# bytedance/particle-sfm

Hardware: AMD Instinct MI355X
Metric: trajectory-points/s (higher is better)
Workload: dtype f32 sampling + f64 positions; 1 GPU; configs[1]: synthetic 100x(1920x1080) flow pairs, sample_ratio=2, flow_check + chaining + occlusion + id assignment, 1 sequence per GPU; frames=101, height=1080, width=1920, trajectories=2073277, parallelism=sequence-per-gpu x1, world_size=1

## Files before the change

### particle-sfm_amd/csrc/psfm_persist.hip

```cpp
#include <hip/hip_ext.h>
#include <stdlib.h>

#include "psfm_internal.h"
#include "psfm_chain.h"

#define PP_BLOCK 256
#define PP_NW (PP_BLOCK / PSFM_WAVE)
#define PP_PROBE 8
#ifndef PP_PRE_WAVES
#define PP_PRE_WAVES 4
#endif
#ifndef PP_KEEP
#define PP_KEEP 0
#endif
#ifndef PP_FC_AHEAD
#define PP_FC_AHEAD 4
#endif
#ifndef PP_FC_FAST
#define PP_FC_FAST 0
#endif
#define PP_GUESTS 32
#ifndef PP_WHATIF
#define PP_WHATIF 0
#endif
#ifndef PP_WAVES_N
#define PP_WAVES_N 8
#endif
#define PP_WAVES __attribute__((amdgpu_waves_per_eu(PP_WAVES_N, PP_WAVES_N)))

#ifdef PSFM_PERSIST_CHECK
#define PP_CHK(idx, lim, code) (((idx) >= 0 && (idx) < (lim)) ? true : (atomicCAS(&a.ctr->pad[0], 0, (code)), atomicMax(&a.ctr->pad[1], (int)(idx)), false))
#else
#define PP_CHK(idx, lim, code) true
#endif
#ifndef PP_COH_MARKS
#define PP_COH_MARKS true
#endif
#define PP_POOLED (-1)
#define PP_PEND (-2)

struct PsfmPersistArgs {
    const float2* flows; const uint8_t* occ;
    const float2* flows_b; uint8_t* occ_w; float thres, t2; int fc; int fc_xcd_per;
    int xcd_per;
    int64_t occ_pitch; PsfmFastDiv wdiv;
    int H, W; float cw, ch, rcw, rch;
    int ratio, GW, GH, G;
    float2* dlog; int cap;
    int cap_main;
    uint8_t* maps;
    unsigned* survsh;
    PsfmCounters* ctr;
    PsfmShard* shards;
    int* free_stack; int free_cap; int nsh;
    unsigned long long* handoff;
    unsigned long long* fin_keys; int* fin_lanes;
    int seg_cap; int spill_base; int spill_cap;
    int2* seg_info;
    unsigned* bar;
    int n_flows, shift_b, shift_d;
    PsfmFastDiv gwdiv, rdiv;
    int spin_limit;
};

struct PsfmFrameView {
    const float2* flow; const uint8_t* occ;
    int H, W; float cw, ch, rcw, rch;
    int ratio, GW, GH;
    uint8_t* blocked_cur; uint8_t stamp_cur;
    PsfmFastDiv rdiv;
};

__device__ __forceinline__ void psfm_put_record(const PsfmPersistArgs& a, int slot, unsigned long long key, int lane)
{
    int64_t o;
    if (slot < a.seg_cap) {
        o = (int64_t)blockIdx.x * a.seg_cap + slot;
    } else {
        const int q = atomicAdd(&a.ctr->spill_cnt, 1);
        if (q >= a.spill_cap) { atomicOr(&a.ctr->overflow, 2); return; }
        o = (int64_t)a.spill_base + q;
    }
    if (!PP_CHK(lane, a.cap, 6)) return;
    a.fin_keys[o] = key;
    a.fin_lanes[o] = lane;
}

__device__ __forceinline__ int psfm_record_slot(int* s_rec_cnt, bool dead)
{
    const unsigned long long dm = __ballot(dead);
    if (dm == 0ull) return 0;
    int base = 0;
    if (psfm_lane_id() == (int)__builtin_ctzll(dm)) base = atomicAdd(s_rec_cnt, __popcll(dm));
    base = __shfl(base, (int)__builtin_ctzll(dm));
    return base + psfm_rank_in(dm);
}

#ifdef PSFM_TIMELINE
__device__ unsigned long long g_pp_tl[2 * 4096 * 8];
__device__ int g_pp_st[4096 * 8];
__device__ int g_pp_tl_frame = -1;
#define PP_TL(k) do { if ((unsigned)(t - g_pp_tl_frame) < 2u && tid == 0) g_pp_tl[((t - g_pp_tl_frame) * 4096 + blockIdx.x) * 8 + (k)] = __builtin_amdgcn_s_memrealtime(); } while (0)
extern "C" int psfm_debug_persist_timeline(int frame, unsigned long long* out_host, int n_blocks)
{
    if (out_host && n_blocks < 0) return hipMemcpyFromSymbol(out_host, HIP_SYMBOL(g_pp_st), (size_t)(-n_blocks) * 32) != hipSuccess;
    if (out_host) return hipMemcpyFromSymbol(out_host, HIP_SYMBOL(g_pp_tl), (size_t)2 * 4096 * 64) != hipSuccess;
    return hipMemcpyToSymbol(HIP_SYMBOL(g_pp_tl_frame), &frame, sizeof(int)) != hipSuccess;
}
#else
#define PP_TL(k) do {} while (0)
#endif

__device__ __forceinline__ void psfm_bar_arrive(const PsfmPersistArgs& a, int shard, int k, int lane)
{
    int last = 0;
    if (lane == 0) {
        const int nblk = (int)gridDim.x;
        const unsigned members = (unsigned)((nblk - shard + PSFM_NSHARD - 1) / PSFM_NSHARD);
        const unsigned old = __hip_atomic_fetch_add(a.bar + shard * 32, 1u, __ATOMIC_RELAXED, __HIP_MEMORY_SCOPE_AGENT);
        if (old + 1 == members * (unsigned)(k + 1)) {
            const unsigned nsh = (unsigned)(nblk < PSFM_NSHARD ? nblk : PSFM_NSHARD);
            const unsigned o2 = __hip_atomic_fetch_add(a.bar + 64 * 32, 1u, __ATOMIC_RELAXED, __HIP_MEMORY_SCOPE_AGENT);
            if (o2 + 1 == nsh * (unsigned)(k + 1)) last = 1;
        }
    }
    last = __builtin_amdgcn_readfirstlane(last);
    if (last) psfm_coh_st(a.bar + (65 + lane) * 32, (unsigned)(k + 1));
}
__device__ __forceinline__ bool psfm_bar_wait(const PsfmPersistArgs& a, int shard, int k)
{
    const unsigned* flag = a.bar + (65 + shard) * 32;
    int n = 0;
    while (psfm_coh_ld(flag) < (unsigned)(k + 1)) {
        __builtin_amdgcn_s_sleep(1);
        if (++n > a.spin_limit) { atomicOr(&a.ctr->overflow, 8); psfm_coh_st(&a.ctr->abort, 1); return false; }
        if ((n & 127) == 0 && psfm_coh_ld(&a.ctr->abort)) return false;
    }
    return true;
}

__device__ __forceinline__ void psfm_fc_slice(const PsfmPersistArgs& a, int f, int tid)
{
    const int P = a.H * a.W;
    PsfmFcParams q;
    q.H = a.H; q.W = a.W; q.cw = a.cw; q.ch = a.ch; q.rcw = a.rcw; q.rch = a.rch; q.thres = a.thres; q.t2 = a.t2;
    const float2* __restrict__ F = a.flows + (size_t)f * P;
    const float2* __restrict__ B = a.flows_b + (size_t)f * P;
    uint8_t* O = a.occ_w + (size_t)f * a.occ_pitch;
    const int nch = (P + 1023) / 1024;
    const int per = a.fc_xcd_per;
    for (int q0 = blockIdx.x; q0 < (per > 0 ? 8 * per : nch); q0 += gridDim.x) {
        const int ci = per > 0 ? (q0 & 7) * per + (q0 >> 3) : q0;
        if (ci >= nch) continue;
        const int p0 = ci * 1024 + tid;
        float2 fv[4];
#pragma unroll
        for (int k = 0; k < 4; ++k) {
            const int p = p0 + k * 256;
            fv[k] = p < P ? psfm_ld(F, (unsigned)p * 8u) : make_float2(0.f, 0.f);
        }
        int y = (int)psfm_fastdiv((unsigned)p0, a.wdiv), x = p0 - y * a.W;
#pragma unroll
        for (int k = 0; k < 4; ++k) {
            const int p = p0 + k * 256;
            if (p >= P) break;
            uint8_t o;
#if PP_FC_FAST
            {
                const float X = __fadd_rn((float)x, fv[k].x), Y = __fadd_rn((float)y, fv[k].y);
                const PsfmTaps t = psfm_taps_t<true>(X, Y, q.cw, q.ch, q.rcw, q.rch, q.H, q.W);
                const bool interior = (t.x0 >= 0) & (t.x0 + 1 < q.W) & (t.y0 >= 0) & (t.y0 + 1 < q.H);
                if (__builtin_amdgcn_ballot_w64(!interior) == 0ull) o = psfm_flow_check_px_interior(B, X, Y, fv[k], t, q);
                else { float e; int xb = x, yb = y; asm volatile("" : "+v"(xb), "+v"(yb)); o = psfm_flow_check_px<false>(B, xb, yb, fv[k], q, &e); }
            }
#else
            float e;
            o = psfm_flow_check_px<false>(B, x, y, fv[k], q, &e);
#endif
            psfm_coh_st(O + p, o);
            x += 256;
            while (x >= a.W) { x -= a.W; ++y; }
        }
    }
}

__device__ __forceinline__ int psfm_vblock(const PsfmPersistArgs& a)
{
    const int b = (int)blockIdx.x;
    return (a.xcd_per > 0 && b < 8 * a.xcd_per) ? (b & 7) * a.xcd_per + (b >> 3) : b;
}

struct PsfmEntry { int kind, ex, host; };

template <int R>
__global__ __launch_bounds__(PP_BLOCK) PP_WAVES void psfm_chain_persist_kernel(PsfmPersistArgs a)
{
    __shared__ int s_births[PP_NW], s_adopt[PP_NW], s_pend[PP_NW];
    __shared__ int s_new_g[PP_BLOCK];
    __shared__ int s_ad_tid[PP_BLOCK];
    __shared__ int s_pend_tid[PP_BLOCK];
    __shared__ double2 s_xp[PP_BLOCK];
    __shared__ int s_xg[PP_BLOCK];
    __shared__ int s_xf[PP_BLOCK];
    __shared__ int s_gi[PP_BLOCK];
    __shared__ int s_npts[PP_BLOCK];
    __shared__ int s_seg_start[PP_PROBE + 1], s_seg_end[PP_PROBE + 1];
    __shared__ int s_nseg, s_base_free, s_ok, s_alive_any[2], s_rec_cnt, s_done;
    __shared__ double2 s_gp[PP_GUESTS];
    __shared__ int s_gbf[PP_GUESTS];
    __shared__ int s_ggi[PP_GUESTS];
    __shared__ int s_glive[PP_GUESTS], s_gfree[PP_GUESTS], s_nglive, s_ngfree;

    int tid = threadIdx.x;
    int L = psfm_vblock(a) * PP_BLOCK + tid;
    const int ratio = R > 0 ? R : a.ratio;
    const int shard = blockIdx.x % PSFM_NSHARD;
    const size_t P = (size_t)a.H * a.W;

    int bf = PP_POOLED;
    double2 p = make_double2(0.0, 0.0);
    s_gi[tid] = L;
    s_npts[tid] = 0;
    if (L < a.G) {
        const int gy = (int)psfm_fastdiv((unsigned)L, a.gwdiv), gx = L - gy * a.GW;
        p = make_double2((double)(gx * ratio), (double)(gy * ratio));
        bf = 0;
        s_npts[tid] = 1;
    }
    s_xf[tid] = 0;
    if (tid < PP_GUESTS) s_gbf[tid] = -1;
    if (tid == 0) { s_rec_cnt = 0; s_alive_any[0] = 0; s_alive_any[1] = 0; s_done = 0; }
    int fc_next = 0;
    if (a.fc) {
        for (; fc_next < 2 && fc_next < a.n_flows; ++fc_next) psfm_fc_slice(a, fc_next, tid);
        __builtin_amdgcn_s_waitcnt(0);
    }
    __syncthreads();
    if (tid / PSFM_WAVE == PP_NW - 1) psfm_bar_arrive(a, shard, 0, tid & (PSFM_WAVE - 1));
    if (a.fc) {
        if (tid == 0) s_ok = psfm_bar_wait(a, shard, 0) ? 1 : 0;
        __syncthreads();
        if (!s_ok) return;
    }

    for (int t = 0; t < a.n_flows; ++t) {
        asm volatile("" : "+v"(tid));
        L = psfm_vblock(a) * PP_BLOCK + tid;
        const int lane = tid & (PSFM_WAVE - 1), wave = tid / PSFM_WAVE;
        PsfmFrameView v;
        v.flow = a.flows + (size_t)t * P; v.occ = a.occ + (size_t)t * a.occ_pitch;
        v.H = a.H; v.W = a.W; v.cw = a.cw; v.ch = a.ch; v.rcw = a.rcw; v.rch = a.rch; v.ratio = a.ratio; v.GW = a.GW; v.GH = a.GH; v.rdiv = a.rdiv;
        v.blocked_cur = a.maps + (size_t)(t % 3) * a.G; v.stamp_cur = 1;
        float2* dlog_t = a.dlog + (size_t)t * a.cap;
        const int cur = t & 1, prev = cur ^ 1;

        PP_TL(0);
        const bool live = bf >= 0;
        bool any_alive = false;
        int npts = 0;
        auto own_step = [&](const PsfmFrameView& vs, float2* slab, int s, const PsfmStepLoads& ld, bool mine, bool& alive_any) {
            PsfmStep s1;
            s1.alive = true;
            if (mine) s1 = psfm_step_finish(vs, p, ld);
            const int slot1 = psfm_record_slot(&s_rec_cnt, !s1.alive);
            if (mine) {
                if (s1.alive) {
                    if (PP_CHK(L, a.cap, 1)) slab[L] = s1.flow;
                    psfm_block_grid<R, PP_COH_MARKS>(vs, (int)s1.next.x, (int)s1.next.y);
                    p = s1.next;
                    alive_any = true;
                    ++npts;
                } else {
                    psfm_put_record(a, slot1, psfm_key(s, bf, s_gi[tid], a.shift_b, a.shift_d), L);
                    bf = PP_PEND;
                    p = make_double2(0.0, 0.0);
                }
            }
        };
        PsfmStepLoads l1 = psfm_step_issue(v, p);

        auto do_E = [&]() { own_step(v, dlog_t, t, l1, live, any_alive); };
        const bool e_first = wave < PP_PRE_WAVES;
        if (e_first) do_E();

        if (a.fc) {
            const unsigned* flag = a.bar + (65 + shard) * 32;
            const int fc_lim = t + PP_FC_AHEAD < a.n_flows ? t + PP_FC_AHEAD : a.n_flows;
            while (fc_next < fc_lim) {
                if (__builtin_amdgcn_readfirstlane((int)psfm_coh_ld(flag)) >= t + 1 || (PP_WHATIF & 32)) break;
                psfm_fc_slice(a, fc_next, tid);
                ++fc_next;
            }
        }
        if (tid == 0) s_ok = (PP_WHATIF & 4) ? 1 : (psfm_bar_wait(a, shard, t) ? 1 : 0);
        __syncthreads();
        if (!s_ok) return;

#ifndef PP_NO_SETPRIO
        __builtin_amdgcn_s_setprio(3);
#endif
        PP_TL(1);
        const bool poll = t > 0 && bf == PP_POOLED && !(PP_WHATIF & 8);
        const bool gridpt = t > 0 && L < a.G && !(PP_WHATIF & 8);
        uint8_t* map_prev = a.maps + (size_t)((t + 2) % 3) * a.G;
        unsigned sv = 0, byte = 0;
        unsigned long long h0 = 0, h1 = 0, h2 = ~0ull;
        if (t > 0 && blockIdx.x == 0 && tid < PSFM_NSHARD) sv = psfm_coh_ld(a.survsh + (prev * PSFM_NSHARD + tid) * 32);
        if (gridpt) byte = psfm_coh_ld(map_prev + L);
        if (poll) {
            const unsigned long long* h = a.handoff + (size_t)L * 3;
            h0 = psfm_coh_ld(h); h1 = psfm_coh_ld(h + 1); h2 = psfm_coh_ld(h + 2);
        }

        if (!e_first) do_E();

        const unsigned long long svm = __ballot(sv == (unsigned)t);
        bool birth = false;
        if (gridpt) {
            if (byte != 0) psfm_coh_st(map_prev + L, (uint8_t)0);
            birth = byte == 0;
            if (L == 0 && svm == 0ull) birth = ((0 + 1) * (0 + 1) + 0 * 0) > ratio * ratio;
            if (PP_WHATIF & 1) birth = false;
        }
        bool adopted = false;
        if (poll) {
            const int tag = (int)(h2 >> 32);
            if ((tag >> 1) == t - 1 && !(PP_WHATIF & 1)) {
                if (tag & 1) {
                    adopted = true;
                    s_xp[tid] = make_double2(__longlong_as_double((long long)h0), __longlong_as_double((long long)h1));
                    s_xg[tid] = (int)(unsigned)h2;
                } else {
                    bf = PP_PEND;
                }
            }
        }
        const bool pend = (bf == PP_PEND) & !live;
        const unsigned long long bm = __ballot(birth), am = __ballot(adopted), pm = __ballot(pend);
        if (lane == 0) { s_births[wave] = __popcll(bm); s_adopt[wave] = __popcll(am); s_pend[wave] = __popcll(pm); }
        if (birth) s_new_g[wave * PSFM_WAVE + psfm_rank_in(bm)] = L;
        if (adopted) s_ad_tid[wave * PSFM_WAVE + psfm_rank_in(am)] = tid;
        if (pend) s_pend_tid[wave * PSFM_WAVE + psfm_rank_in(pm)] = tid;
        if (wave == 0) {
            const int gb = tid < PP_GUESTS ? s_gbf[tid] : -1;
            const bool gl = gb >= 0, gf = (tid < PP_GUESTS) & (gb < 0);
            const unsigned long long glm = __ballot(gl), gfm = __ballot(gf);
            if (lane == 0) { s_nglive = __popcll(glm); s_ngfree = __popcll(gfm); }
            if (gl) s_glive[psfm_rank_in(glm)] = tid;
            if (gf) s_gfree[psfm_rank_in(gfm)] = tid;
        }
        __syncthreads();

        PP_TL(2);
        int nb = 0, nad = 0, npd = 0, my_pend_before = 0;
#pragma unroll
        for (int w = 0; w < PP_NW; ++w) {
            if (w == wave) my_pend_before = npd;
            nb += s_births[w]; nad += s_adopt[w]; npd += s_pend[w];
        }
        const int matched = nb < npd ? nb : npd;
        const int ngl = s_nglive;
        const int gmatched = (nb - matched) < s_ngfree ? (nb - matched) : s_ngfree;
        const int n2 = nb + nad + ngl;

        for (int base = 0; base == 0 || base < n2; base += PP_BLOCK) {
            const int k = base + tid;
            PsfmEntry e;
            e.kind = 0; e.ex = -1; e.host = -1;
            if (k < nb) {
                int before = 0, pb = 0;
#pragma unroll
                for (int w = 0; w < PP_NW; ++w) {
                    const int c = s_births[w], pc = s_pend[w];
                    if (k >= before && k < before + c) e.ex = s_new_g[w * PSFM_WAVE + (k - before)];
                    if (k >= pb && k < pb + pc) e.host = s_pend_tid[w * PSFM_WAVE + (k - pb)];
                    before += c; pb += pc;
                }
                e.kind = 1;
            } else if (k < nb + nad) {
                const int kk = k - nb;
                int before = 0;
#pragma unroll
                for (int w = 0; w < PP_NW; ++w) {
                    const int c = s_adopt[w];
                    if (kk >= before && kk < before + c) e.ex = s_ad_tid[w * PSFM_WAVE + (kk - before)];
                    before += c;
                }
                e.kind = 2;
            } else if (k < n2) {
                e.ex = s_glive[k - nb - nad];
                e.kind = 3;
            }
            PsfmStepLoads l2 = {};
            if (e.kind != 0) {
                double2 q;
                if (e.kind == 1) {
                    const int gy = (int)psfm_fastdiv((unsigned)e.ex, a.gwdiv), gx = e.ex - gy * a.GW;
                    q = make_double2((double)(gx * ratio), (double)(gy * ratio));
                } else if (e.kind == 2) {
                    q = s_xp[e.ex];
                } else {
                    q = s_gp[e.ex];
                }
                l2 = psfm_step_issue(v, q);
            }
#ifdef PSFM_TIMELINE
            if (base == 0 && tid == 0 && t == g_pp_tl_frame) {
                int* st = g_pp_st + blockIdx.x * 8;
                st[0] = nb; st[1] = nad; st[2] = npd; st[3] = ngl; st[4] = s_ngfree; st[5] = nb - matched - gmatched; st[6] = npd - matched - PP_KEEP;
            }
#endif
            if (base == 0 && tid == 0) {
                PsfmShard* sh_pop = a.shards + cur * PSFM_NSHARD;
                PsfmShard* sh_push = a.shards + prev * PSFM_NSHARD;
                int need = nb - matched - gmatched;
                const int n_push = npd - matched - PP_KEEP;
                int bfree = 0;
                const int fsh = blockIdx.x % a.nsh;
                if (n_push > 0) bfree = atomicAdd(&sh_push[fsh].free_top, n_push);
                int nseg = 0, done = 0;
                for (int rd = 0; rd < PP_PROBE / 4 && need > 0; ++rd) {
                    const int q4 = need >> 2, r4 = need & 3;
                    int sh[4], ask[4], old[4];
#pragma unroll
                    for (int j = 0; j < 4; ++j) {
                        sh[j] = (fsh + (rd * 4 + j) * 7) % a.nsh;
                        ask[j] = q4 + (j < r4 ? 1 : 0);
                        old[j] = ask[j] > 0 ? atomicSub(&sh_pop[sh[j]].free_top, ask[j]) : 0;
                    }
#pragma unroll
                    for (int j = 0; j < 4; ++j) {
                        const int take = old[j] < 0 ? 0 : (old[j] > ask[j] ? ask[j] : old[j]);
                        if (take < ask[j]) atomicAdd(&sh_pop[sh[j]].free_top, ask[j] - take);
                        if (take > 0) {
                            s_seg_start[nseg] = sh[j] * a.free_cap + old[j] - 1;
                            done += take;
                            s_seg_end[nseg] = done;
                            ++nseg;
                            need -= take;
                        }
                    }
                }
                s_base_free = bfree;
                if (need > 0) {
                    const int base_new = atomicAdd(&a.ctr->n_lanes, need);
                    s_seg_start[nseg] = -(base_new + 1);
                    done += need;
                    s_seg_end[nseg] = done;
                    ++nseg;
                }
                s_nseg = nseg;
            }
            PP_TL(3);
            __syncthreads();
            PP_TL(4);

            if (base == 0) {
                if (pend) {
                    const int r = my_pend_before + psfm_rank_in(pm);
                    if (r >= matched + PP_KEEP) {
                        int* free_push = a.free_stack + (size_t)prev * a.free_cap * PSFM_NSHARD;
                        const int fpos = s_base_free + (r - matched - PP_KEEP);
                        if (fpos < a.free_cap && PP_CHK(fpos, a.free_cap, 7)) psfm_coh_st(free_push + (size_t)(blockIdx.x % a.nsh) * a.free_cap + fpos, L);
                        else atomicOr(&a.ctr->overflow, 1);
                        bf = PP_POOLED;
                    }
                }
            }
            psfm_step_pin<true>(l2);
            asm volatile("" : "+v"(e.ex));
            if (e.kind != 0) {
                double2 q;
                int bfk, gik, col, gs = -1;
                if (e.kind == 1) {
                    const int gy = (int)psfm_fastdiv((unsigned)e.ex, a.gwdiv), gx = e.ex - gy * a.GW;
                    q = make_double2((double)(gx * ratio), (double)(gy * ratio));
                    bfk = t; gik = e.ex;
                    if (k < matched) {
                        col = psfm_vblock(a) * PP_BLOCK + e.host;
                    } else if (k < matched + gmatched) {
                        gs = s_gfree[k - matched];
                        col = a.cap_main + blockIdx.x * PP_GUESTS + gs;
                    } else {
                        const int* free_pop = a.free_stack + (size_t)cur * a.free_cap * PSFM_NSHARD;
                        const int qq = k - matched - gmatched;
                        int j = 0, pv = 0;
                        while (j < s_nseg - 1 && qq >= s_seg_end[j]) { pv = s_seg_end[j]; ++j; }
                        const int st = s_seg_start[j];
                        if (st >= 0) (void)PP_CHK(st - (qq - pv), 2 * a.free_cap * PSFM_NSHARD, 9);
                        col = st >= 0 ? psfm_coh_ld(free_pop + (st - (qq - pv))) : (-(st + 1) + (qq - pv));
                        if (col >= a.cap_main) col = -1;
                    }
                } else if (e.kind == 2) {
                    q = s_xp[e.ex];
                    bfk = t - 1; gik = s_xg[e.ex];
                    col = psfm_vblock(a) * PP_BLOCK + e.ex;
                } else {
                    q = s_gp[e.ex];
                    bfk = s_gbf[e.ex]; gik = s_ggi[e.ex];
                    col = a.cap_main + blockIdx.x * PP_GUESTS + e.ex;
                }
                if (col >= 0) {
                    (void)PP_CHK(col, a.cap, 2);
                    const PsfmStep s2 = psfm_step_finish(v, q, l2);
                    if (e.kind == 1) ++npts;
                    if (s2.alive) {
                        if (PP_CHK(col, a.cap, 3)) dlog_t[col] = s2.flow;
                        psfm_block_grid<R, PP_COH_MARKS>(v, (int)s2.next.x, (int)s2.next.y);
                        any_alive = true;
                        ++npts;
                    } else {
                        const int slot = atomicAdd(&s_rec_cnt, 1);
                        psfm_put_record(a, slot, psfm_key(t, bfk, gik, a.shift_b, a.shift_d), col);
                    }
                    if (e.kind == 1) {
                        const bool popped = k >= matched + gmatched;
                        if (popped && s2.alive && t == a.n_flows - 1) {
                            const int slot = atomicAdd(&s_rec_cnt, 1);
                            psfm_put_record(a, slot, psfm_key(a.n_flows, t, e.ex, a.shift_b, a.shift_d), col);
                        }
                        if (k < matched) {
                            s_xp[e.host] = s2.next; s_xg[e.host] = e.ex; s_xf[e.host] = s2.alive ? 1 : 2;
                        } else if (gs >= 0) {
                            if (s2.alive) { s_gp[gs] = s2.next; s_ggi[gs] = e.ex; s_gbf[gs] = t; }
                        } else if (PP_CHK(col, a.cap_main, 8)) {
                            unsigned long long* h = a.handoff + (size_t)col * 3;
                            psfm_coh_st(h, (unsigned long long)__double_as_longlong(s2.next.x));
                            psfm_coh_st(h + 1, (unsigned long long)__double_as_longlong(s2.next.y));
                            psfm_coh_st(h + 2, (unsigned long long)(unsigned)e.ex |
                                                   ((unsigned long long)(unsigned)(2 * t + (s2.alive ? 1 : 0)) << 32));
                        }
                    } else if (e.kind == 2) {
                        if (s2.alive) s_xp[e.ex] = s2.next;
                        s_xf[e.ex] = s2.alive ? 1 : 2;
                    } else {
                        if (s2.alive) s_gp[e.ex] = s2.next;
                        else s_gbf[e.ex] = -1;
                    }
                } else {
                    atomicOr(&a.ctr->overflow, 4);
                }
            }
        }
        PP_TL(5);
        if (npts) s_npts[tid] += npts;
        const unsigned long long alm = __ballot(any_alive);
        if (lane == 0 && alm != 0ull) s_alive_any[t & 1] = 1;
        __syncthreads();
        {
            const int f = s_xf[tid];
            if (f != 0) {
                s_xf[tid] = 0;
                if (f == 1) {
                    bf = adopted ? t - 1 : t;
                    s_gi[tid] = s_xg[tid];
                    p = s_xp[tid];
                } else {
                    bf = PP_PEND;
                }
            }
        }
        if (tid == 0 && s_alive_any[t & 1]) { psfm_coh_st(a.survsh + (cur * PSFM_NSHARD + shard) * 32, (unsigned)(t + 1)); s_alive_any[t & 1] = 0; }
        if (a.fc) {
            const int need = t + 3 < a.n_flows ? t + 3 : a.n_flows;
            if (!(PP_WHATIF & 16)) for (; fc_next < need; ++fc_next) psfm_fc_slice(a, fc_next, tid);
        }
        if (!(PP_WHATIF & 2)) asm volatile("s_waitcnt vmcnt(0) lgkmcnt(0)" ::: "memory");
        PP_TL(6);
        {
            int last_wave = 0;
            if (lane == 0) last_wave = atomicAdd(&s_done, 1) == PP_NW - 1 ? 1 : 0;
            last_wave = __builtin_amdgcn_readfirstlane(last_wave);
            if (last_wave) {
                if (lane == 0) s_done = 0;
                PP_TL(7);
                psfm_bar_arrive(a, shard, t + 1, lane);
            }
        }
#ifndef PP_NO_SETPRIO
        __builtin_amdgcn_s_setprio(0);
#endif
    }

    const int lane = tid & (PSFM_WAVE - 1), wave = tid / PSFM_WAVE;
    {
        const bool alive = bf >= 0;
        const int slot = psfm_record_slot(&s_rec_cnt, alive);
        if (alive) psfm_put_record(a, slot, psfm_key(a.n_flows, bf, s_gi[tid], a.shift_b, a.shift_d), L);
        if (tid < PP_GUESTS && s_gbf[tid] >= 0) {
            const int gslot = atomicAdd(&s_rec_cnt, 1);
            psfm_put_record(a, gslot, psfm_key(a.n_flows, s_gbf[tid], s_ggi[tid], a.shift_b, a.shift_d),
                            a.cap_main + blockIdx.x * PP_GUESTS + tid);
        }
    }
    {
        __shared__ int s_pts[PP_NW];
        int w = s_npts[tid];
#pragma unroll
        for (int o = 32; o > 0; o >>= 1) w += __shfl_down(w, o);
        if (lane == 0) s_pts[wave] = w;
        __syncthreads();
        if (tid == 0) {
            int tot = 0;
            for (int j = 0; j < PP_NW; ++j) tot += s_pts[j];
            const int c = s_rec_cnt;
            a.seg_info[blockIdx.x] = make_int2(c < a.seg_cap ? c : a.seg_cap, tot);
        }
    }
}

__global__ __launch_bounds__(256) void psfm_persist_init_kernel(PsfmCounters* ctr, PsfmShard* shards, int G,
                                                                unsigned long long* maps64, size_t n_maps64,
                                                                unsigned long long* bar64, size_t n_bar64,
                                                                unsigned long long* handoff, size_t n_handoff)
{
    const size_t i = (size_t)blockIdx.x * 256 + threadIdx.x, stride = (size_t)gridDim.x * 256;
    if (i == 0) { ctr->n_lanes = G; ctr->overflow = 0; ctr->stall = 0; ctr->abort = 0; ctr->spill_cnt = 0; ctr->pad[0] = 0; ctr->pad[1] = 0; }
    if (i < 2 * PSFM_NSHARD) { shards[i].fin_cnt = 0; shards[i].free_top = 0; shards[i].points = 0u; }
    for (size_t k = i; k < n_maps64; k += stride) maps64[k] = 0ull;
    for (size_t k = i; k < n_bar64; k += stride) bar64[k] = 0ull;
    for (size_t k = i; k < n_handoff; k += stride) handoff[k] = ~0ull;
}

int psfm_persist_guests(void) { return PP_GUESTS; }

int psfm_persist_max_blocks(psfm_ctx* c)
{
    if (c->persist_max_blocks >= 0) return c->persist_max_blocks;
    int cus = 0;
    c->persist_max_blocks = 0;
    if (hipDeviceGetAttribute(&cus, hipDeviceAttributeMultiprocessorCount, c->device) != hipSuccess) {
        (void)hipGetLastError();
        return 0;
    }
    int per_cu = 1 << 30;
    const void* inst[4] = {(const void*)psfm_chain_persist_kernel<0>, (const void*)psfm_chain_persist_kernel<1>,
                           (const void*)psfm_chain_persist_kernel<2>, (const void*)psfm_chain_persist_kernel<4>};
    for (int k = 0; k < 4; ++k) {
        int v = 0;
        if (hipOccupancyMaxActiveBlocksPerMultiprocessor(&v, inst[k], PP_BLOCK, 0) != hipSuccess) {
            (void)hipGetLastError();
            return 0;
        }
        per_cu = v < per_cu ? v : per_cu;
    }
    if (per_cu > 8) per_cu = 8;
    c->persist_max_blocks = per_cu * cus;
    return c->persist_max_blocks;
}

psfm_status psfm_launch_chain_persist(psfm_ctx* c, const PsfmTrackDims& d, const float* flows, const uint8_t* occ,
                                      int64_t occ_pitch, const float* flows_b, float thres, hipStream_t s)
{
    const size_t bar_bytes = (size_t)(4 * PSFM_NSHARD + 1) * 128;
    {
        const size_t n_maps64 = ((size_t)d.G * 3 + 7) / 8, n_bar64 = bar_bytes / 8, n_handoff = (size_t)d.nblk * PP_BLOCK * 3;
        hipLaunchKernelGGL(psfm_persist_init_kernel, dim3(1024), dim3(256), 0, s, c->counters.as<PsfmCounters>(),
                           c->shards.as<PsfmShard>(), (int)d.G, c->occupied.as<unsigned long long>(), n_maps64,
                           c->persist_bar.as<unsigned long long>(), n_bar64, c->handoff.as<unsigned long long>(), n_handoff);
    }
    PsfmPersistArgs a;
    a.flows = (const float2*)flows; a.occ = occ;
    a.occ_pitch = occ_pitch;
    a.flows_b = (const float2*)flows_b; a.occ_w = const_cast<uint8_t*>(occ); a.thres = thres; a.t2 = psfm_sq_threshold(thres); a.fc = flows_b != nullptr;
    {
        static const int xcd_on = getenv("PSFM_FC_XCD") ? atoi(getenv("PSFM_FC_XCD")) : 1;
        const int64_t nch = ((int64_t)d.H * d.W + 1023) / 1024;
        a.fc_xcd_per = xcd_on && nch >= 64 ? (int)((nch + 7) / 8) : 0;
    }
    {
        static const int pp_xcd = getenv("PSFM_PP_XCD") ? atoi(getenv("PSFM_PP_XCD")) : 1;
        const int64_t gb = (d.G + PP_BLOCK - 1) / PP_BLOCK;
        const int per = (int)((gb + 7) / 8);
        a.xcd_per = (pp_xcd && gb >= 64 && 8 * per <= d.nblk) ? per : 0;
    }
    a.wdiv = psfm_fastdiv_make((unsigned)d.W);
    a.H = d.H; a.W = d.W; a.cw = d.cw; a.ch = d.ch; a.rcw = psfm_rcp_host(d.cw); a.rch = psfm_rcp_host(d.ch);
    a.ratio = d.ratio; a.GW = d.GW; a.GH = d.GH; a.G = (int)d.G;
    a.dlog = c->log.as<float2>(); a.cap = (int)d.cap; a.cap_main = d.nblk * PP_BLOCK;
    a.maps = c->occupied.as<uint8_t>();
    a.ctr = c->counters.as<PsfmCounters>();
    a.shards = c->shards.as<PsfmShard>();
    a.free_stack = c->free_stack.as<int>(); a.free_cap = d.free_cap; a.nsh = d.nsh;
    a.handoff = c->handoff.as<unsigned long long>();
    a.fin_keys = c->fin_keys.as<unsigned long long>(); a.fin_lanes = c->fin_lanes.as<int>();
    a.seg_cap = d.seg_cap; a.spill_base = d.nblk * d.seg_cap; a.spill_cap = d.spill_cap;
    a.seg_info = c->seg_info.as<int2>();
    a.bar = c->persist_bar.as<unsigned>();
    a.survsh = a.bar + (2 * PSFM_NSHARD + 1) * 32;
    a.n_flows = d.n_flows; a.shift_b = d.shift_b; a.shift_d = d.shift_d;
    a.gwdiv = psfm_fastdiv_make((unsigned)d.GW); a.rdiv = psfm_fastdiv_make((unsigned)d.ratio);
    a.spin_limit = 1 << 18;
    if (const char* e = getenv("PSFM_PERSIST_SPIN_LIMIT")) a.spin_limit = atoi(e);
    hipEvent_t e0 = nullptr, e1 = nullptr;
    c->prof.kernel_span(PSFM_PROF_CHAIN, &e0, &e1, true);
    const dim3 grid((unsigned)d.nblk), block(PP_BLOCK);
    const bool coop = getenv("PSFM_PERSIST_COOP") && atoi(getenv("PSFM_PERSIST_COOP")) != 0;
    const void* fn = d.ratio == 1 ? (const void*)psfm_chain_persist_kernel<1> : d.ratio == 2 ? (const void*)psfm_chain_persist_kernel<2>
                   : d.ratio == 4 ? (const void*)psfm_chain_persist_kernel<4> : (const void*)psfm_chain_persist_kernel<0>;
    if (coop) {
        void* kargs[] = {(void*)&a};
        if (e0) PSFM_HIP(hipEventRecord(e0, s));
        const hipError_t le = hipLaunchCooperativeKernel(fn, grid, block, kargs, 0, s);
        if (le != hipSuccess) {
            (void)hipGetLastError();
            psfm_set_error("cooperative launch of the persistent frame loop refused: %s", hipGetErrorString(le));
            return PSFM_ERR_CAPACITY;
        }
        if (e1) PSFM_HIP(hipEventRecord(e1, s));
        return PSFM_OK;
    }
    switch (d.ratio) {
        case 1: hipExtLaunchKernelGGL(psfm_chain_persist_kernel<1>, grid, block, 0, s, e0, e1, 0, a); break;
        case 2: hipExtLaunchKernelGGL(psfm_chain_persist_kernel<2>, grid, block, 0, s, e0, e1, 0, a); break;
        case 4: hipExtLaunchKernelGGL(psfm_chain_persist_kernel<4>, grid, block, 0, s, e0, e1, 0, a); break;
        default: hipExtLaunchKernelGGL(psfm_chain_persist_kernel<0>, grid, block, 0, s, e0, e1, 0, a); break;
    }
    PSFM_HIP(hipGetLastError());
    return PSFM_OK;
}
```

Baseline: 20.99 billion trajectory-points/s.

## Split persistent kernel args into hot/cold and reload from kernarg segment

Splits the kernel argument struct into a hot part and a cold part and reads fields straight from the kernarg segment pointer at each use, instead of keeping the whole argument struct live in scalar registers across the frame loop. Empty asm barriers on block id, t and tid keep them in SGPRs, which is meant to cut register pressure in the waves_per_eu-constrained persistent kernel. It also reworks the adoption flag encoding (PP_DIED, f==3) and splits the frame view into a frame part and a marks part. The cost is repeated scalar loads from kernarg memory, and there is some risk that the state-encoding changes alter behavior.

```diff
diff --git a/particle-sfm_amd/csrc/psfm_persist.hip b/particle-sfm_amd/csrc/psfm_persist.hip
--- a/particle-sfm_amd/csrc/psfm_persist.hip
+++ b/particle-sfm_amd/csrc/psfm_persist.hip
@@ -29,7 +29,7 @@
 #define PP_WAVES __attribute__((amdgpu_waves_per_eu(PP_WAVES_N, PP_WAVES_N)))
 
 #ifdef PSFM_PERSIST_CHECK
-#define PP_CHK(idx, lim, code) (((idx) >= 0 && (idx) < (lim)) ? true : (atomicCAS(&a.ctr->pad[0], 0, (code)), atomicMax(&a.ctr->pad[1], (int)(idx)), false))
+#define PP_CHK(idx, lim, code) (((idx) >= 0 && (idx) < (lim)) ? true : (atomicCAS(&psfm_cold()->ctr->pad[0], 0, (code)), atomicMax(&psfm_cold()->ctr->pad[1], (int)(idx)), false))
 #else
 #define PP_CHK(idx, lim, code) true
 #endif
@@ -38,52 +38,122 @@
 #endif
 #define PP_POOLED (-1)
 #define PP_PEND (-2)
+#define PP_DIED (-3)
 
 struct PsfmPersistArgs {
-    const float2* flows; const uint8_t* occ;
-    const float2* flows_b; uint8_t* occ_w; float thres, t2; int fc; int fc_xcd_per;
+    const float2* flows; uint8_t* occ;
+    const float2* flows_b; float t2; int fc; int fc_xcd_per;
     int xcd_per;
     int64_t occ_pitch; PsfmFastDiv wdiv;
     int H, W; float cw, ch, rcw, rch;
     int ratio, GW, GH, G;
     float2* dlog; int cap;
+    uint8_t* maps;
+    unsigned long long* handoff;
+    unsigned* bar;
+    int n_flows;
+    int nblk;
+    PsfmFastDiv gwdiv, rdiv;
+};
+#define PP_SURV ((2 * PSFM_NSHARD + 1) * 32)
+
+struct PsfmPersistCold {
     int cap_main;
-    uint8_t* maps;
-    unsigned* survsh;
+    int cap;
     PsfmCounters* ctr;
     PsfmShard* shards;
     int* free_stack; int free_cap; int nsh;
-    unsigned long long* handoff;
     unsigned long long* fin_keys; int* fin_lanes;
     int seg_cap; int spill_base; int spill_cap;
     int2* seg_info;
-    unsigned* bar;
-    int n_flows, shift_b, shift_d;
-    PsfmFastDiv gwdiv, rdiv;
+    int shift_b, shift_d;
     int spin_limit;
 };
+struct PsfmPersistKernarg { PsfmPersistArgs hot; PsfmPersistCold cold; };
+
+typedef const __attribute__((address_space(4))) PsfmPersistArgs* PsfmHotPtr;
+typedef const __attribute__((address_space(4))) PsfmPersistCold* PsfmColdPtr;
+__device__ __forceinline__ PsfmHotPtr psfm_hot()
+{
+    const __attribute__((address_space(4))) char* k = (const __attribute__((address_space(4))) char*)__builtin_amdgcn_kernarg_segment_ptr();
+    asm volatile("" : "+s"(k));
+    return (PsfmHotPtr)(k + offsetof(PsfmPersistKernarg, hot));
+}
+#define PA psfm_hot()
+__device__ __forceinline__ int psfm_bid()
+{
+    int b = (int)blockIdx.x;
+    asm volatile("" : "+s"(b));
+    return b;
+}
+#define PP_BID psfm_bid()
+#define PP_SHARD (psfm_bid() & (PSFM_NSHARD - 1))
+template <class P> __device__ __forceinline__ PsfmFastDiv psfm_fd(P p)
+{
+    PsfmFastDiv f;
+    f.m = p->m; f.sh1 = p->sh1; f.sh2 = p->sh2; f.d = 0u;
+    return f;
+}
+__device__ __forceinline__ PsfmColdPtr psfm_cold()
+{
+    const __attribute__((address_space(4))) char* k = (const __attribute__((address_space(4))) char*)__builtin_amdgcn_kernarg_segment_ptr();
+    asm volatile("" : "+s"(k));
+    return (PsfmColdPtr)(k + offsetof(PsfmPersistKernarg, cold));
+}
 
 struct PsfmFrameView {
     const float2* flow; const uint8_t* occ;
     int H, W; float cw, ch, rcw, rch;
+};
+struct PsfmMarksView {
     int ratio, GW, GH;
     uint8_t* blocked_cur; uint8_t stamp_cur;
     PsfmFastDiv rdiv;
+    float2* slab;
 };
 
-__device__ __forceinline__ void psfm_put_record(const PsfmPersistArgs& a, int slot, unsigned long long key, int lane)
-{
+__device__ __forceinline__ PsfmFrameView psfm_frame_view(int t)
+{
+    const PsfmHotPtr a = psfm_hot();
+    PsfmFrameView v;
+    v.H = a->H; v.W = a->W; v.cw = a->cw; v.ch = a->ch; v.rcw = a->rcw; v.rch = a->rch;
+    v.flow = a->flows + (size_t)t * ((size_t)v.H * v.W); v.occ = a->occ + (size_t)t * a->occ_pitch;
+    return v;
+}
+template <int R>
+__device__ __forceinline__ PsfmMarksView psfm_marks_view(int t)
+{
+    const PsfmHotPtr a = psfm_hot();
+    PsfmMarksView m;
+    m.ratio = R > 0 ? R : a->ratio; m.GW = a->GW; m.GH = a->GH;
+    if (R > 0) { m.rdiv.m = 0u; m.rdiv.sh1 = 0; m.rdiv.sh2 = 0; m.rdiv.d = 0u; }
+    else m.rdiv = psfm_fd(&a->rdiv);
+    m.blocked_cur = a->maps + (size_t)(t % 3) * a->G; m.stamp_cur = 1;
+    m.slab = a->dlog + (size_t)t * a->cap;
+    return m;
+}
+
+__device__ __forceinline__ void psfm_put_record(int slot, unsigned long long key, int lane)
+{
+    const PsfmColdPtr c = psfm_cold();
+    const int seg_cap = c->seg_cap;
     int64_t o;
-    if (slot < a.seg_cap) {
-        o = (int64_t)blockIdx.x * a.seg_cap + slot;
+    if (slot < seg_cap) {
+        o = (int64_t)PP_BID * seg_cap + slot;
     } else {
-        const int q = atomicAdd(&a.ctr->spill_cnt, 1);
-        if (q >= a.spill_cap) { atomicOr(&a.ctr->overflow, 2); return; }
-        o = (int64_t)a.spill_base + q;
-    }
-    if (!PP_CHK(lane, a.cap, 6)) return;
-    a.fin_keys[o] = key;
-    a.fin_lanes[o] = lane;
+        PsfmCounters* ctr = c->ctr;
+        const int q = atomicAdd(&ctr->spill_cnt, 1);
+        if (q >= c->spill_cap) { atomicOr(&ctr->overflow, 2); return; }
+        o = (int64_t)c->spill_base + q;
+    }
+    if (!PP_CHK(lane, c->cap, 6)) return;
+    c->fin_keys[o] = key;
+    c->fin_lanes[o] = lane;
+}
+__device__ __forceinline__ unsigned long long psfm_cold_key(int last_time, int bf, int idx)
+{
+    const PsfmColdPtr c = psfm_cold();
+    return psfm_key(last_time, bf, idx, c->shift_b, c->shift_d);
 }
 
 __device__ __forceinline__ int psfm_record_slot(int* s_rec_cnt, bool dead)
@@ -111,45 +181,49 @@
 #define PP_TL(k) do {} while (0)
 #endif
 
-__device__ __forceinline__ void psfm_bar_arrive(const PsfmPersistArgs& a, int shard, int k, int lane)
+__device__ __forceinline__ void psfm_bar_arrive(int shard, int k, int lane)
 {
     int last = 0;
+    asm volatile("" : "+s"(k));
     if (lane == 0) {
-        const int nblk = (int)gridDim.x;
+        const int nblk = PA->nblk;
         const unsigned members = (unsigned)((nblk - shard + PSFM_NSHARD - 1) / PSFM_NSHARD);
-        const unsigned old = __hip_atomic_fetch_add(a.bar + shard * 32, 1u, __ATOMIC_RELAXED, __HIP_MEMORY_SCOPE_AGENT);
+        const unsigned old = __hip_atomic_fetch_add(PA->bar + shard * 32, 1u, __ATOMIC_RELAXED, __HIP_MEMORY_SCOPE_AGENT);
         if (old + 1 == members * (unsigned)(k + 1)) {
             const unsigned nsh = (unsigned)(nblk < PSFM_NSHARD ? nblk : PSFM_NSHARD);
-            const unsigned o2 = __hip_atomic_fetch_add(a.bar + 64 * 32, 1u, __ATOMIC_RELAXED, __HIP_MEMORY_SCOPE_AGENT);
+            const unsigned o2 = __hip_atomic_fetch_add(PA->bar + 64 * 32, 1u, __ATOMIC_RELAXED, __HIP_MEMORY_SCOPE_AGENT);
             if (o2 + 1 == nsh * (unsigned)(k + 1)) last = 1;
         }
     }
     last = __builtin_amdgcn_readfirstlane(last);
-    if (last) psfm_coh_st(a.bar + (65 + lane) * 32, (unsigned)(k + 1));
-}
-__device__ __forceinline__ bool psfm_bar_wait(const PsfmPersistArgs& a, int shard, int k)
-{
-    const unsigned* flag = a.bar + (65 + shard) * 32;
+    if (last) psfm_coh_st(PA->bar + (65 + lane) * 32, (unsigned)(k + 1));
+}
+__device__ __forceinline__ bool psfm_bar_wait(int shard, int k)
+{
+    const unsigned* flag = PA->bar + (65 + shard) * 32;
     int n = 0;
     while (psfm_coh_ld(flag) < (unsigned)(k + 1)) {
         __builtin_amdgcn_s_sleep(1);
-        if (++n > a.spin_limit) { atomicOr(&a.ctr->overflow, 8); psfm_coh_st(&a.ctr->abort, 1); return false; }
-        if ((n & 127) == 0 && psfm_coh_ld(&a.ctr->abort)) return false;
+        if (++n > psfm_cold()->spin_limit) { PsfmCounters* ctr = psfm_cold()->ctr; atomicOr(&ctr->overflow, 8); psfm_coh_st(&ctr->abort, 1); return false; }
+        if ((n & 127) == 0 && psfm_coh_ld(&psfm_cold()->ctr->abort)) return false;
     }
     return true;
 }
 
-__device__ __forceinline__ void psfm_fc_slice(const PsfmPersistArgs& a, int f, int tid)
-{
-    const int P = a.H * a.W;
+__device__ __forceinline__ void psfm_fc_slice(int f, int tid)
+{
+    const PsfmHotPtr a = psfm_hot();
+    const int P = a->H * a->W;
     PsfmFcParams q;
-    q.H = a.H; q.W = a.W; q.cw = a.cw; q.ch = a.ch; q.rcw = a.rcw; q.rch = a.rch; q.thres = a.thres; q.t2 = a.t2;
-    const float2* __restrict__ F = a.flows + (size_t)f * P;
-    const float2* __restrict__ B = a.flows_b + (size_t)f * P;
-    uint8_t* O = a.occ_w + (size_t)f * a.occ_pitch;
+    q.H = a->H; q.W = a->W; q.cw = a->cw; q.ch = a->ch; q.rcw = a->rcw; q.rch = a->rch; q.thres = 0.f ; q.t2 = a->t2;
+    const float2* __restrict__ F = a->flows + (size_t)f * P;
+    const float2* __restrict__ B = a->flows_b + (size_t)f * P;
+    uint8_t* O = a->occ + (size_t)f * a->occ_pitch;
+    const PsfmFastDiv wdiv = psfm_fd(&a->wdiv);
+    const int W = a->W;
     const int nch = (P + 1023) / 1024;
-    const int per = a.fc_xcd_per;
-    for (int q0 = blockIdx.x; q0 < (per > 0 ? 8 * per : nch); q0 += gridDim.x) {
+    const int per = a->fc_xcd_per, nblk = a->nblk;
+    for (int q0 = PP_BID; q0 < (per > 0 ? 8 * per : nch); q0 += nblk) {
         const int ci = per > 0 ? (q0 & 7) * per + (q0 >> 3) : q0;
         if (ci >= nch) continue;
         const int p0 = ci * 1024 + tid;
@@ -159,7 +233,7 @@
             const int p = p0 + k * 256;
             fv[k] = p < P ? psfm_ld(F, (unsigned)p * 8u) : make_float2(0.f, 0.f);
         }
-        int y = (int)psfm_fastdiv((unsigned)p0, a.wdiv), x = p0 - y * a.W;
+        int y = (int)psfm_fastdiv((unsigned)p0, wdiv), x = p0 - y * W;
 #pragma unroll
         for (int k = 0; k < 4; ++k) {
             const int p = p0 + k * 256;
@@ -179,21 +253,21 @@
 #endif
             psfm_coh_st(O + p, o);
             x += 256;
-            while (x >= a.W) { x -= a.W; ++y; }
-        }
-    }
-}
-
-__device__ __forceinline__ int psfm_vblock(const PsfmPersistArgs& a)
-{
-    const int b = (int)blockIdx.x;
-    return (a.xcd_per > 0 && b < 8 * a.xcd_per) ? (b & 7) * a.xcd_per + (b >> 3) : b;
+            while (x >= W) { x -= W; ++y; }
+        }
+    }
+}
+
+__device__ __forceinline__ int psfm_vblock()
+{
+    const int b = PP_BID, per = PA->xcd_per;
+    return (per > 0 && b < 8 * per) ? (b & 7) * per + (b >> 3) : b;
 }
 
 struct PsfmEntry { int kind, ex, host; };
 
 template <int R>
-__global__ __launch_bounds__(PP_BLOCK) PP_WAVES void psfm_chain_persist_kernel(PsfmPersistArgs a)
+__global__ __launch_bounds__(PP_BLOCK) PP_WAVES void psfm_chain_persist_kernel(PsfmPersistKernarg)
 {
     __shared__ int s_births[PP_NW], s_adopt[PP_NW], s_pend[PP_NW];
     __shared__ int s_new_g[PP_BLOCK];
@@ -212,17 +286,16 @@
     __shared__ int s_glive[PP_GUESTS], s_gfree[PP_GUESTS], s_nglive, s_ngfree;
 
     int tid = threadIdx.x;
-    int L = psfm_vblock(a) * PP_BLOCK + tid;
-    const int ratio = R > 0 ? R : a.ratio;
-    const int shard = blockIdx.x % PSFM_NSHARD;
-    const size_t P = (size_t)a.H * a.W;
+    int L = psfm_vblock() * PP_BLOCK + tid;
+    const int ratio = R > 0 ? R : PA->ratio;
 
     int bf = PP_POOLED;
     double2 p = make_double2(0.0, 0.0);
     s_gi[tid] = L;
     s_npts[tid] = 0;
-    if (L < a.G) {
-        const int gy = (int)psfm_fastdiv((unsigned)L, a.gwdiv), gx = L - gy * a.GW;
+    if (L < PA->G) {
+        const PsfmHotPtr a = psfm_hot();
+        const int gy = (int)psfm_fastdiv((unsigned)L, psfm_fd(&a->gwdiv)), gx = L - gy * a->GW;
         p = make_double2((double)(gx * ratio), (double)(gy * ratio));
         bf = 0;
         s_npts[tid] = 1;
@@ -231,68 +304,66 @@
     if (tid < PP_GUESTS) s_gbf[tid] = -1;
     if (tid == 0) { s_rec_cnt = 0; s_alive_any[0] = 0; s_alive_any[1] = 0; s_done = 0; }
     int fc_next = 0;
-    if (a.fc) {
-        for (; fc_next < 2 && fc_next < a.n_flows; ++fc_next) psfm_fc_slice(a, fc_next, tid);
+    if (PA->fc) {
+        for (; fc_next < 2 && fc_next < PA->n_flows; ++fc_next) psfm_fc_slice(fc_next, tid);
         __builtin_amdgcn_s_waitcnt(0);
     }
     __syncthreads();
-    if (tid / PSFM_WAVE == PP_NW - 1) psfm_bar_arrive(a, shard, 0, tid & (PSFM_WAVE - 1));
-    if (a.fc) {
-        if (tid == 0) s_ok = psfm_bar_wait(a, shard, 0) ? 1 : 0;
+    if (tid / PSFM_WAVE == PP_NW - 1) psfm_bar_arrive(PP_SHARD, 0, tid & (PSFM_WAVE - 1));
+    if (PA->fc) {
+        if (tid == 0) s_ok = psfm_bar_wait(PP_SHARD, 0) ? 1 : 0;
         __syncthreads();
         if (!s_ok) return;
     }
 
-    for (int t = 0; t < a.n_flows; ++t) {
+    for (int t = 0; t < PA->n_flows; ++t) {
         asm volatile("" : "+v"(tid));
-        L = psfm_vblock(a) * PP_BLOCK + tid;
+        L = psfm_vblock() * PP_BLOCK + tid;
         const int lane = tid & (PSFM_WAVE - 1), wave = tid / PSFM_WAVE;
-        PsfmFrameView v;
-        v.flow = a.flows + (size_t)t * P; v.occ = a.occ + (size_t)t * a.occ_pitch;
-        v.H = a.H; v.W = a.W; v.cw = a.cw; v.ch = a.ch; v.rcw = a.rcw; v.rch = a.rch; v.ratio = a.ratio; v.GW = a.GW; v.GH = a.GH; v.rdiv = a.rdiv;
-        v.blocked_cur = a.maps + (size_t)(t % 3) * a.G; v.stamp_cur = 1;
-        float2* dlog_t = a.dlog + (size_t)t * a.cap;
+        PsfmFrameView v = psfm_frame_view(t);
         const int cur = t & 1, prev = cur ^ 1;
 
         PP_TL(0);
         const bool live = bf >= 0;
         bool any_alive = false;
         int npts = 0;
-        auto own_step = [&](const PsfmFrameView& vs, float2* slab, int s, const PsfmStepLoads& ld, bool mine, bool& alive_any) {
+        auto own_step = [&](const PsfmFrameView& vs, int s, const PsfmStepLoads& ld, bool mine, bool& alive_any) {
             PsfmStep s1;
             s1.alive = true;
             if (mine) s1 = psfm_step_finish(vs, p, ld);
             const int slot1 = psfm_record_slot(&s_rec_cnt, !s1.alive);
             if (mine) {
                 if (s1.alive) {
-                    if (PP_CHK(L, a.cap, 1)) slab[L] = s1.flow;
-                    psfm_block_grid<R, PP_COH_MARKS>(vs, (int)s1.next.x, (int)s1.next.y);
+                    const PsfmMarksView m = psfm_marks_view<R>(s);
+                    if (PP_CHK(L, PA->cap, 1)) m.slab[L] = s1.flow;
+                    psfm_block_grid<R, PP_COH_MARKS>(m, (int)s1.next.x, (int)s1.next.y);
                     p = s1.next;
                     alive_any = true;
                     ++npts;
                 } else {
-                    psfm_put_record(a, slot1, psfm_key(s, bf, s_gi[tid], a.shift_b, a.shift_d), L);
-                    bf = PP_PEND;
+                    psfm_put_record(slot1, psfm_cold_key(s, bf, s_gi[tid]), L);
+                    bf = PP_DIED;
                     p = make_double2(0.0, 0.0);
                 }
             }
         };
         PsfmStepLoads l1 = psfm_step_issue(v, p);
 
-        auto do_E = [&]() { own_step(v, dlog_t, t, l1, live, any_alive); };
+        auto do_E = [&]() { own_step(v, t, l1, live, any_alive); };
         const bool e_first = wave < PP_PRE_WAVES;
         if (e_first) do_E();
 
-        if (a.fc) {
-            const unsigned* flag = a.bar + (65 + shard) * 32;
-            const int fc_lim = t + PP_FC_AHEAD < a.n_flows ? t + PP_FC_AHEAD : a.n_flows;
+        if (PA->fc) {
+            const PsfmHotPtr a = psfm_hot();
+            const unsigned* flag = a->bar + (65 + PP_SHARD) * 32;
+            const int nf = a->n_flows, fc_lim = t + PP_FC_AHEAD < nf ? t + PP_FC_AHEAD : nf;
             while (fc_next < fc_lim) {
                 if (__builtin_amdgcn_readfirstlane((int)psfm_coh_ld(flag)) >= t + 1 || (PP_WHATIF & 32)) break;
-                psfm_fc_slice(a, fc_next, tid);
+                psfm_fc_slice(fc_next, tid);
                 ++fc_next;
             }
         }
-        if (tid == 0) s_ok = (PP_WHATIF & 4) ? 1 : (psfm_bar_wait(a, shard, t) ? 1 : 0);
+        if (tid == 0) s_ok = (PP_WHATIF & 4) ? 1 : (psfm_bar_wait(PP_SHARD, t) ? 1 : 0);
         __syncthreads();
         if (!s_ok) return;
 
@@ -301,17 +372,20 @@
 #endif
         PP_TL(1);
         const bool poll = t > 0 && bf == PP_POOLED && !(PP_WHATIF & 8);
-        const bool gridpt = t > 0 && L < a.G && !(PP_WHATIF & 8);
-        uint8_t* map_prev = a.maps + (size_t)((t + 2) % 3) * a.G;
+        const PsfmHotPtr ac = psfm_hot();
+        const int G = ac->G;
+        const bool gridpt = t > 0 && L < G && !(PP_WHATIF & 8);
+        uint8_t* map_prev = ac->maps + (size_t)((t + 2) % 3) * G;
         unsigned sv = 0, byte = 0;
         unsigned long long h0 = 0, h1 = 0, h2 = ~0ull;
-        if (t > 0 && blockIdx.x == 0 && tid < PSFM_NSHARD) sv = psfm_coh_ld(a.survsh + (prev * PSFM_NSHARD + tid) * 32);
+        if (t > 0 && PP_BID == 0 && tid < PSFM_NSHARD) sv = psfm_coh_ld(ac->bar + PP_SURV + (prev * PSFM_NSHARD + tid) * 32);
         if (gridpt) byte = psfm_coh_ld(map_prev + L);
         if (poll) {
-            const unsigned long long* h = a.handoff + (size_t)L * 3;
+            const unsigned long long* h = ac->handoff + (size_t)L * 3;
             h0 = psfm_coh_ld(h); h1 = psfm_coh_ld(h + 1); h2 = psfm_coh_ld(h + 2);
         }
 
+        v = psfm_frame_view(t);
         if (!e_first) do_E();
 
         const unsigned long long svm = __ballot(sv == (unsigned)t);
@@ -319,7 +393,10 @@
         if (gridpt) {
             if (byte != 0) psfm_coh_st(map_prev + L, (uint8_t)0);
             birth = byte == 0;
-            if (L == 0 && svm == 0ull) birth = ((0 + 1) * (0 + 1) + 0 * 0) > ratio * ratio;
+            if (L == 0 && svm == 0ull) {
+                const int r0 = R > 0 ? R : PA->ratio;
+                birth = ((0 + 1) * (0 + 1) + 0 * 0) > r0 * r0;
+            }
             if (PP_WHATIF & 1) birth = false;
         }
         bool adopted = false;
@@ -335,7 +412,8 @@
                 }
             }
         }
-        const bool pend = (bf == PP_PEND) & !live;
+        const bool pend = bf == PP_PEND;
+        if (bf == PP_DIED) bf = PP_PEND;
         const unsigned long long bm = __ballot(birth), am = __ballot(adopted), pm = __ballot(pend);
         if (lane == 0) { s_births[wave] = __popcll(bm); s_adopt[wave] = __popcll(am); s_pend[wave] = __popcll(pm); }
         if (birth) s_new_g[wave * PSFM_WAVE + psfm_rank_in(bm)] = L;
@@ -362,8 +440,13 @@
         const int ngl = s_nglive;
         const int gmatched = (nb - matched) < s_ngfree ? (nb - matched) : s_ngfree;
         const int n2 = nb + nad + ngl;
+        const int t_frame = t, nb_f = __builtin_amdgcn_readfirstlane(nb), nad_f = __builtin_amdgcn_readfirstlane(nad), npd_f = __builtin_amdgcn_readfirstlane(npd),
+                  matched_f = __builtin_amdgcn_readfirstlane(matched), gmatched_f = __builtin_amdgcn_readfirstlane(gmatched);
 
         for (int base = 0; base == 0 || base < n2; base += PP_BLOCK) {
+            int t = t_frame, nb = nb_f, nad = nad_f, npd = npd_f, matched = matched_f, gmatched = gmatched_f;
+            asm volatile("" : "+s"(t), "+s"(nb), "+s"(nad), "+s"(npd), "+s"(matched), "+s"(gmatched));
+            const int cur = t & 1, prev = cur ^ 1;
             const int k = base + tid;
             PsfmEntry e;
             e.kind = 0; e.ex = -1; e.host = -1;
@@ -395,7 +478,8 @@
             if (e.kind != 0) {
                 double2 q;
                 if (e.kind == 1) {
-                    const int gy = (int)psfm_fastdiv((unsigned)e.ex, a.gwdiv), gx = e.ex - gy * a.GW;
+                    const PsfmHotPtr a = psfm_hot();
+                    const int gy = (int)psfm_fastdiv((unsigned)e.ex, psfm_fd(&a->gwdiv)), gx = e.ex - gy * a->GW;
                     q = make_double2((double)(gx * ratio), (double)(gy * ratio));
                 } else if (e.kind == 2) {
                     q = s_xp[e.ex];
@@ -406,17 +490,19 @@
             }
 #ifdef PSFM_TIMELINE
             if (base == 0 && tid == 0 && t == g_pp_tl_frame) {
-                int* st = g_pp_st + blockIdx.x * 8;
+                int* st = g_pp_st + PP_BID * 8;
                 st[0] = nb; st[1] = nad; st[2] = npd; st[3] = ngl; st[4] = s_ngfree; st[5] = nb - matched - gmatched; st[6] = npd - matched - PP_KEEP;
             }
 #endif
             if (base == 0 && tid == 0) {
-                PsfmShard* sh_pop = a.shards + cur * PSFM_NSHARD;
-                PsfmShard* sh_push = a.shards + prev * PSFM_NSHARD;
+                const PsfmColdPtr c = psfm_cold();
+                const int nsh = c->nsh, free_cap = c->free_cap;
+                PsfmShard* sh_pop = c->shards + cur * PSFM_NSHARD;
+                PsfmShard* sh_push = c->shards + prev * PSFM_NSHARD;
                 int need = nb - matched - gmatched;
                 const int n_push = npd - matched - PP_KEEP;
                 int bfree = 0;
-                const int fsh = blockIdx.x % a.nsh;
+                const int fsh = PP_BID % nsh;
                 if (n_push > 0) bfree = atomicAdd(&sh_push[fsh].free_top, n_push);
                 int nseg = 0, done = 0;
                 for (int rd = 0; rd < PP_PROBE / 4 && need > 0; ++rd) {
@@ -424,7 +510,7 @@
                     int sh[4], ask[4], old[4];
 #pragma unroll
                     for (int j = 0; j < 4; ++j) {
-                        sh[j] = (fsh + (rd * 4 + j) * 7) % a.nsh;
+                        sh[j] = (fsh + (rd * 4 + j) * 7) % nsh;
                         ask[j] = q4 + (j < r4 ? 1 : 0);
                         old[j] = ask[j] > 0 ? atomicSub(&sh_pop[sh[j]].free_top, ask[j]) : 0;
                     }
@@ -433,7 +519,7 @@
                         const int take = old[j] < 0 ? 0 : (old[j] > ask[j] ? ask[j] : old[j]);
                         if (take < ask[j]) atomicAdd(&sh_pop[sh[j]].free_top, ask[j] - take);
                         if (take > 0) {
-                            s_seg_start[nseg] = sh[j] * a.free_cap + old[j] - 1;
+                            s_seg_start[nseg] = sh[j] * free_cap + old[j] - 1;
                             done += take;
                             s_seg_end[nseg] = done;
                             ++nseg;
@@ -443,7 +529,7 @@
                 }
                 s_base_free = bfree;
                 if (need > 0) {
-                    const int base_new = atomicAdd(&a.ctr->n_lanes, need);
+                    const int base_new = atomicAdd(&c->ctr->n_lanes, need);
                     s_seg_start[nseg] = -(base_new + 1);
                     done += need;
                     s_seg_end[nseg] = done;
@@ -459,10 +545,12 @@
                 if (pend) {
                     const int r = my_pend_before + psfm_rank_in(pm);
                     if (r >= matched + PP_KEEP) {
-                        int* free_push = a.free_stack + (size_t)prev * a.free_cap * PSFM_NSHARD;
+                        const PsfmColdPtr c = psfm_cold();
+                        const int free_cap = c->free_cap;
+                        int* free_push = c->free_stack + (size_t)prev * free_cap * PSFM_NSHARD;
                         const int fpos = s_base_free + (r - matched - PP_KEEP);
-                        if (fpos < a.free_cap && PP_CHK(fpos, a.free_cap, 7)) psfm_coh_st(free_push + (size_t)(blockIdx.x % a.nsh) * a.free_cap + fpos, L);
-                        else atomicOr(&a.ctr->overflow, 1);
+                        if (fpos < free_cap && PP_CHK(fpos, free_cap, 7)) psfm_coh_st(free_push + (size_t)(PP_BID % c->nsh) * free_cap + fpos, L);
+                        else atomicOr(&c->ctr->overflow, 1);
                         bf = PP_POOLED;
                     }
                 }
@@ -473,58 +561,62 @@
                 double2 q;
                 int bfk, gik, col, gs = -1;
                 if (e.kind == 1) {
-                    const int gy = (int)psfm_fastdiv((unsigned)e.ex, a.gwdiv), gx = e.ex - gy * a.GW;
+                    const PsfmHotPtr a = psfm_hot();
+                    const int gy = (int)psfm_fastdiv((unsigned)e.ex, psfm_fd(&a->gwdiv)), gx = e.ex - gy * a->GW;
                     q = make_double2((double)(gx * ratio), (double)(gy * ratio));
                     bfk = t; gik = e.ex;
                     if (k < matched) {
-                        col = psfm_vblock(a) * PP_BLOCK + e.host;
+                        col = psfm_vblock() * PP_BLOCK + e.host;
                     } else if (k < matched + gmatched) {
                         gs = s_gfree[k - matched];
-                        col = a.cap_main + blockIdx.x * PP_GUESTS + gs;
+                        col = psfm_cold()->cap_main + PP_BID * PP_GUESTS + gs;
                     } else {
-                        const int* free_pop = a.free_stack + (size_t)cur * a.free_cap * PSFM_NSHARD;
+                        const PsfmColdPtr c = psfm_cold();
+                        const int* free_pop = c->free_stack + (size_t)cur * c->free_cap * PSFM_NSHARD;
                         const int qq = k - matched - gmatched;
                         int j = 0, pv = 0;
                         while (j < s_nseg - 1 && qq >= s_seg_end[j]) { pv = s_seg_end[j]; ++j; }
                         const int st = s_seg_start[j];
-                        if (st >= 0) (void)PP_CHK(st - (qq - pv), 2 * a.free_cap * PSFM_NSHARD, 9);
+                        if (st >= 0) (void)PP_CHK(st - (qq - pv), 2 * c->free_cap * PSFM_NSHARD, 9);
                         col = st >= 0 ? psfm_coh_ld(free_pop + (st - (qq - pv))) : (-(st + 1) + (qq - pv));
-                        if (col >= a.cap_main) col = -1;
+                        if (col >= c->cap_main) col = -1;
                     }
                 } else if (e.kind == 2) {
                     q = s_xp[e.ex];
                     bfk = t - 1; gik = s_xg[e.ex];
-                    col = psfm_vblock(a) * PP_BLOCK + e.ex;
+                    col = psfm_vblock() * PP_BLOCK + e.ex;
                 } else {
                     q = s_gp[e.ex];
                     bfk = s_gbf[e.ex]; gik = s_ggi[e.ex];
-                    col = a.cap_main + blockIdx.x * PP_GUESTS + e.ex;
+                    col = psfm_cold()->cap_main + PP_BID * PP_GUESTS + e.ex;
                 }
                 if (col >= 0) {
-                    (void)PP_CHK(col, a.cap, 2);
+                    (void)PP_CHK(col, PA->cap, 2);
                     const PsfmStep s2 = psfm_step_finish(v, q, l2);
                     if (e.kind == 1) ++npts;
                     if (s2.alive) {
-                        if (PP_CHK(col, a.cap, 3)) dlog_t[col] = s2.flow;
-                        psfm_block_grid<R, PP_COH_MARKS>(v, (int)s2.next.x, (int)s2.next.y);
+                        const PsfmMarksView m = psfm_marks_view<R>(t);
+                        if (PP_CHK(col, PA->cap, 3)) m.slab[col] = s2.flow;
+                        psfm_block_grid<R, PP_COH_MARKS>(m, (int)s2.next.x, (int)s2.next.y);
                         any_alive = true;
                         ++npts;
                     } else {
                         const int slot = atomicAdd(&s_rec_cnt, 1);
-                        psfm_put_record(a, slot, psfm_key(t, bfk, gik, a.shift_b, a.shift_d), col);
+                        psfm_put_record(slot, psfm_cold_key(t, bfk, gik), col);
                     }
                     if (e.kind == 1) {
                         const bool popped = k >= matched + gmatched;
-                        if (popped && s2.alive && t == a.n_flows - 1) {
+                        const int nf = PA->n_flows;
+                        if (popped && s2.alive && t == nf - 1) {
                             const int slot = atomicAdd(&s_rec_cnt, 1);
-                            psfm_put_record(a, slot, psfm_key(a.n_flows, t, e.ex, a.shift_b, a.shift_d), col);
+                            psfm_put_record(slot, psfm_cold_key(nf, t, e.ex), col);
                         }
                         if (k < matched) {
                             s_xp[e.host] = s2.next; s_xg[e.host] = e.ex; s_xf[e.host] = s2.alive ? 1 : 2;
                         } else if (gs >= 0) {
                             if (s2.alive) { s_gp[gs] = s2.next; s_ggi[gs] = e.ex; s_gbf[gs] = t; }
-                        } else if (PP_CHK(col, a.cap_main, 8)) {
-                            unsigned long long* h = a.handoff + (size_t)col * 3;
+                        } else if (PP_CHK(col, psfm_cold()->cap_main, 8)) {
+                            unsigned long long* h = PA->handoff + (size_t)col * 3;
                             psfm_coh_st(h, (unsigned long long)__double_as_longlong(s2.next.x));
                             psfm_coh_st(h + 1, (unsigned long long)__double_as_longlong(s2.next.y));
                             psfm_coh_st(h + 2, (unsigned long long)(unsigned)e.ex |
@@ -532,17 +624,18 @@
                         }
                     } else if (e.kind == 2) {
                         if (s2.alive) s_xp[e.ex] = s2.next;
-                        s_xf[e.ex] = s2.alive ? 1 : 2;
+                        s_xf[e.ex] = s2.alive ? 3 : 2;
                     } else {
                         if (s2.alive) s_gp[e.ex] = s2.next;
                         else s_gbf[e.ex] = -1;
                     }
                 } else {
-                    atomicOr(&a.ctr->overflow, 4);
+                    atomicOr(&psfm_cold()->ctr->overflow, 4);
                 }
             }
         }
         PP_TL(5);
+        asm volatile("" : "+s"(t), "+v"(tid));
         if (npts) s_npts[tid] += npts;
         const unsigned long long alm = __ballot(any_alive);
         if (lane == 0 && alm != 0ull) s_alive_any[t & 1] = 1;
@@ -551,8 +644,8 @@
             const int f = s_xf[tid];
             if (f != 0) {
                 s_xf[tid] = 0;
-                if (f == 1) {
-                    bf = adopted ? t - 1 : t;
+                if (f != 2) {
+                    bf = f == 3 ? t - 1 : t;
                     s_gi[tid] = s_xg[tid];
                     p = s_xp[tid];
                 } else {
@@ -560,10 +653,10 @@
                 }
             }
         }
-        if (tid == 0 && s_alive_any[t & 1]) { psfm_coh_st(a.survsh + (cur * PSFM_NSHARD + shard) * 32, (unsigned)(t + 1)); s_alive_any[t & 1] = 0; }
-        if (a.fc) {
-            const int need = t + 3 < a.n_flows ? t + 3 : a.n_flows;
-            if (!(PP_WHATIF & 16)) for (; fc_next < need; ++fc_next) psfm_fc_slice(a, fc_next, tid);
+        if (tid == 0 && s_alive_any[t & 1]) { psfm_coh_st(PA->bar + PP_SURV + ((t & 1) * PSFM_NSHARD + PP_SHARD) * 32, (unsigned)(t + 1)); s_alive_any[t & 1] = 0; }
+        if (PA->fc) {
+            const int nf = PA->n_flows, need = t + 3 < nf ? t + 3 : nf;
+            if (!(PP_WHATIF & 16)) for (; fc_next < need; ++fc_next) psfm_fc_slice(fc_next, tid);
         }
         if (!(PP_WHATIF & 2)) asm volatile("s_waitcnt vmcnt(0) lgkmcnt(0)" ::: "memory");
         PP_TL(6);
@@ -574,7 +667,7 @@
             if (last_wave) {
                 if (lane == 0) s_done = 0;
                 PP_TL(7);
-                psfm_bar_arrive(a, shard, t + 1, lane);
+                psfm_bar_arrive(PP_SHARD, t + 1, lane);
             }
         }
 #ifndef PP_NO_SETPRIO
@@ -584,13 +677,14 @@
 
     const int lane = tid & (PSFM_WAVE - 1), wave = tid / PSFM_WAVE;
     {
+        const int nf = PA->n_flows;
         const bool alive = bf >= 0;
         const int slot = psfm_record_slot(&s_rec_cnt, alive);
-        if (alive) psfm_put_record(a, slot, psfm_key(a.n_flows, bf, s_gi[tid], a.shift_b, a.shift_d), L);
+        if (alive) psfm_put_record(slot, psfm_cold_key(nf, bf, s_gi[tid]), L);
         if (tid < PP_GUESTS && s_gbf[tid] >= 0) {
             const int gslot = atomicAdd(&s_rec_cnt, 1);
-            psfm_put_record(a, gslot, psfm_key(a.n_flows, s_gbf[tid], s_ggi[tid], a.shift_b, a.shift_d),
-                            a.cap_main + blockIdx.x * PP_GUESTS + tid);
+            psfm_put_record(gslot, psfm_cold_key(nf, s_gbf[tid], s_ggi[tid]),
+                            psfm_cold()->cap_main + PP_BID * PP_GUESTS + tid);
         }
     }
     {
@@ -604,7 +698,9 @@
             int tot = 0;
             for (int j = 0; j < PP_NW; ++j) tot += s_pts[j];
             const int c = s_rec_cnt;
-            a.seg_info[blockIdx.x] = make_int2(c < a.seg_cap ? c : a.seg_cap, tot);
+            const PsfmColdPtr cold = psfm_cold();
+            const int seg_cap = cold->seg_cap;
+            cold->seg_info[PP_BID] = make_int2(c < seg_cap ? c : seg_cap, tot);
         }
     }
 }
@@ -659,10 +755,12 @@
                            c->shards.as<PsfmShard>(), (int)d.G, c->occupied.as<unsigned long long>(), n_maps64,
                            c->persist_bar.as<unsigned long long>(), n_bar64, c->handoff.as<unsigned long long>(), n_handoff);
     }
-    PsfmPersistArgs a;
-    a.flows = (const float2*)flows; a.occ = occ;
+    PsfmPersistKernarg ka;
+    PsfmPersistArgs& a = ka.hot;
+    PsfmPersistCold& k = ka.cold;
+    a.flows = (const float2*)flows; a.occ = const_cast<uint8_t*>(occ);
     a.occ_pitch = occ_pitch;
-    a.flows_b = (const float2*)flows_b; a.occ_w = const_cast<uint8_t*>(occ); a.thres = thres; a.t2 = psfm_sq_threshold(thres); a.fc = flows_b != nullptr;
+    a.flows_b = (const float2*)flows_b; a.t2 = psfm_sq_threshold(thres); a.fc = flows_b != nullptr;
     {
         static const int xcd_on = getenv("PSFM_FC_XCD") ? atoi(getenv("PSFM_FC_XCD")) : 1;
         const int64_t nch = ((int64_t)d.H * d.W + 1023) / 1024;
@@ -677,21 +775,20 @@
     a.wdiv = psfm_fastdiv_make((unsigned)d.W);
     a.H = d.H; a.W = d.W; a.cw = d.cw; a.ch = d.ch; a.rcw = psfm_rcp_host(d.cw); a.rch = psfm_rcp_host(d.ch);
     a.ratio = d.ratio; a.GW = d.GW; a.GH = d.GH; a.G = (int)d.G;
-    a.dlog = c->log.as<float2>(); a.cap = (int)d.cap; a.cap_main = d.nblk * PP_BLOCK;
+    a.dlog = c->log.as<float2>(); a.cap = k.cap = (int)d.cap; k.cap_main = d.nblk * PP_BLOCK;
     a.maps = c->occupied.as<uint8_t>();
-    a.ctr = c->counters.as<PsfmCounters>();
-    a.shards = c->shards.as<PsfmShard>();
-    a.free_stack = c->free_stack.as<int>(); a.free_cap = d.free_cap; a.nsh = d.nsh;
+    k.ctr = c->counters.as<PsfmCounters>();
+    k.shards = c->shards.as<PsfmShard>();
+    k.free_stack = c->free_stack.as<int>(); k.free_cap = d.free_cap; k.nsh = d.nsh;
     a.handoff = c->handoff.as<unsigned long long>();
-    a.fin_keys = c->fin_keys.as<unsigned long long>(); a.fin_lanes = c->fin_lanes.as<int>();
-    a.seg_cap = d.seg_cap; a.spill_base = d.nblk * d.seg_cap; a.spill_cap = d.spill_cap;
-    a.seg_info = c->seg_info.as<int2>();
+    k.fin_keys = c->fin_keys.as<unsigned long long>(); k.fin_lanes = c->fin_lanes.as<int>();
+    k.seg_cap = d.seg_cap; k.spill_base = d.nblk * d.seg_cap; k.spill_cap = d.spill_cap;
+    k.seg_info = c->seg_info.as<int2>();
     a.bar = c->persist_bar.as<unsigned>();
-    a.survsh = a.bar + (2 * PSFM_NSHARD + 1) * 32;
-    a.n_flows = d.n_flows; a.shift_b = d.shift_b; a.shift_d = d.shift_d;
+    a.n_flows = d.n_flows; a.nblk = d.nblk; k.shift_b = d.shift_b; k.shift_d = d.shift_d;
     a.gwdiv = psfm_fastdiv_make((unsigned)d.GW); a.rdiv = psfm_fastdiv_make((unsigned)d.ratio);
-    a.spin_limit = 1 << 18;
-    if (const char* e = getenv("PSFM_PERSIST_SPIN_LIMIT")) a.spin_limit = atoi(e);
+    k.spin_limit = 1 << 18;
+    if (const char* e = getenv("PSFM_PERSIST_SPIN_LIMIT")) k.spin_limit = atoi(e);
     hipEvent_t e0 = nullptr, e1 = nullptr;
     c->prof.kernel_span(PSFM_PROF_CHAIN, &e0, &e1, true);
     const dim3 grid((unsigned)d.nblk), block(PP_BLOCK);
@@ -699,7 +796,7 @@
     const void* fn = d.ratio == 1 ? (const void*)psfm_chain_persist_kernel<1> : d.ratio == 2 ? (const void*)psfm_chain_persist_kernel<2>
                    : d.ratio == 4 ? (const void*)psfm_chain_persist_kernel<4> : (const void*)psfm_chain_persist_kernel<0>;
     if (coop) {
-        void* kargs[] = {(void*)&a};
+        void* kargs[] = {(void*)&ka};
         if (e0) PSFM_HIP(hipEventRecord(e0, s));
         const hipError_t le = hipLaunchCooperativeKernel(fn, grid, block, kargs, 0, s);
         if (le != hipSuccess) {
@@ -711,10 +808,10 @@
         return PSFM_OK;
     }
     switch (d.ratio) {
-        case 1: hipExtLaunchKernelGGL(psfm_chain_persist_kernel<1>, grid, block, 0, s, e0, e1, 0, a); break;
-        case 2: hipExtLaunchKernelGGL(psfm_chain_persist_kernel<2>, grid, block, 0, s, e0, e1, 0, a); break;
-        case 4: hipExtLaunchKernelGGL(psfm_chain_persist_kernel<4>, grid, block, 0, s, e0, e1, 0, a); break;
-        default: hipExtLaunchKernelGGL(psfm_chain_persist_kernel<0>, grid, block, 0, s, e0, e1, 0, a); break;
+        case 1: hipExtLaunchKernelGGL(psfm_chain_persist_kernel<1>, grid, block, 0, s, e0, e1, 0, ka); break;
+        case 2: hipExtLaunchKernelGGL(psfm_chain_persist_kernel<2>, grid, block, 0, s, e0, e1, 0, ka); break;
+        case 4: hipExtLaunchKernelGGL(psfm_chain_persist_kernel<4>, grid, block, 0, s, e0, e1, 0, ka); break;
+        default: hipExtLaunchKernelGGL(psfm_chain_persist_kernel<0>, grid, block, 0, s, e0, e1, 0, ka); break;
     }
     PSFM_HIP(hipGetLastError());
     return PSFM_OK;
```

Measured after the change: 21.82 billion trajectory-points/s, median of 6. 1.04x the previous value.
